# Derek-TH-Wang/OpenRoboRL

Hardware: AMD Instinct MI355X
Metric: env steps/sec at N parallel robots (higher is better)
Workload: dtype f32

## Files before the change

openroborl_amd/csrc/orr_device.h:

```cpp
#pragma once
#include <hip/hip_runtime.h>
#include <stddef.h>
#include <stdint.h>

#include "../../include/openroborl_hip.h"

#define ORR_PI_F 3.14159265358979323846f
#define WSYNC()                             \
  do {                                      \
    asm volatile("" ::: "memory");          \
    __builtin_amdgcn_wave_barrier();        \
    asm volatile("" ::: "memory");          \
  } while (0)

namespace orr {

constexpr int kLanes = 16;
constexpr int kRPW = 64 / kLanes;
constexpr int kMaxRows = 28;
constexpr int kHead = 308;

struct DevClip {
  const float* frames;
  const float* vels;
  int F, flags;
  double dt_d, dur_d;
  double sim_dt_d;
  float cdp[3];
  float cdh;
};
static_assert(sizeof(DevClip) == 64, "clip header = 16 words");

struct ModelHot {
  float jdir[12], joff[12];
  float joint_lo[12], joint_hi[12];
  float joint_pos[12][3];
  float toe_pos[4][3];
  float shank_pos[4][3];
  float lower_com[4][3];
  float init_quat[4];
  float toe_radius, shank_radius;
  float contact_cfm, contact_erp_dt;
};
static_assert(sizeof(ModelHot) == 512, "LDS budget: 4 robots per wave, two waves per SIMD = 20 KB per wave (DESIGN.md section 3)");
struct ModelCold {
  float init_pos[3];
  float foot_friction;
  float init_motor_angles[12], motor_dir[12], motor_offset[12];
  int joint_of_motor[12];
  float kp[12], kd[12];
  float tau_sign[12];
  float tau_sign_motor[12];
  float link_com[12][3];
  float default_joints[12];
  int num_fall;
  int fall_body[ORR_MAX_FALL_PROXIES];
  float fall_pos[ORR_MAX_FALL_PROXIES][3];
  float fall_radius[ORR_MAX_FALL_PROXIES];
  float mass[13];
  float inertia[13][6];
  float inertia_pa[13][6];
  int group[13];
  int friction_anchor;
};
struct alignas(16) DevModel {
  ModelHot hot;
  ModelCold cold;
};
static_assert(sizeof(DevModel) % 16 == 0 && offsetof(DevModel, hot) == 0, "16-byte pieces");
constexpr int kModelLdsWords = (int)(sizeof(ModelHot) / 4);

struct DevTables {
  DevModel model[ORR_MAX_ROBOT_TYPES];
  DevClip clip[ORR_MAX_CLIPS];
  int clip_set[ORR_MAX_ROBOT_TYPES][ORR_MAX_CLIPS];
  int clip_set_n[ORR_MAX_ROBOT_TYPES];
  int* clip_log;
  float clip_switch[ORR_MAX_ROBOT_TYPES][2];
  orr_task_noise noise;
};
static_assert(sizeof(orr_task_noise) == 32, "the noise variants read it as eight words");

struct ReplayArgs {
  const float* traj;
  const float* eff;
  const uint8_t* fall;
  float* tau_out;
  const float* uniforms;
};

struct KParams {
  orr_config cfg;
  float fb[3], fa[3];
  const DevTables* tab;
  float* state;
  long long* counters;
  float* ep_log;
  int ep_log_cap;
  int simds;
  int anchor_on;
#ifdef ORR_WAVE_TIMELINE
  long long* wave_times;
// ... 332 lines not shown
```

openroborl_amd/csrc/orr_env_kernels.h:

```cpp
#pragma once
#if defined(ORR_PHASE_TIMERS) && !defined(ORR_WAVE_TIMELINE)
#define ORR_WAVE_TIMELINE 1
#endif
#ifndef ORR_TU_MAIN
#undef ORR_PHASE_TIMERS
#endif
#include <hip/hip_runtime.h>
#include <type_traits>
#include <math.h>
#include <stdint.h>
#include <stdio.h>
#include <stdlib.h>
#include <string.h>

#include "orr_device.h"

#ifdef ORR_PHASE_TIMERS
__device__ long long g_phase_cycles[orr::kPhaseSlots];
__device__ long long g_wave_phases[2048 * 40];
#define PT_INIT() do { if (threadIdx.x == 0) { for (int i_ = 0; i_ < orr::kPhaseSlots; i_++) S.pt_acc[i_] = 0; S.pt_last = clock64(); } } while (0)
#define PT(k) do { if (threadIdx.x == 0) { const long long t_ = clock64(); S.pt_acc[k] += t_ - S.pt_last; S.pt_last = clock64(); } } while (0)
#define PT_FLUSH() do { if (threadIdx.x == 0 && blockIdx.x == gridDim.x / 2) for (int i_ = 0; i_ < orr::kPhaseSlots; i_++) atomicAdd((unsigned long long*)&g_phase_cycles[i_], (unsigned long long)S.pt_acc[i_]); \
                        if (threadIdx.x == 0 && blockIdx.x < 2048) for (int i_ = 0; i_ < orr::kPhaseSlots; i_++) g_wave_phases[blockIdx.x * 40 + i_] = S.pt_acc[i_]; } while (0)
#else
// ... 79 lines not shown
  }
  for (int i = lane; i < kMaxRows * kWStride; i += kLanes) (&S.ph.sub.W[0][0])[i] = 0.0f;
  WSYNC();
  LegConst K;
  load_leg_const(P, S, lane, K);
  {
    float rel[4], Rb[9];
    base_rotation(S, lane, rel, Rb);
  }
  AnchorState AS = {{0.0f, 0.0f, 0.0f}, {0.0f, 0.0f, 0.0f}, 0};
  bool anchor_robot = false;
  const int aleg = lane < 4 ? lane : (lane < 8 ? lane - 4 : (lane - 8) >> 1);
  if constexpr (ANCHOR) {
    static_assert(kLanes == 16, "ANCHOR: aleg indexes the record's four cached points by the 16-lane row layout");
    anchor_robot = model_cold(P, geti(S, O(ROBOT_TYPE)))->friction_anchor != 0;
    const float* an = rec + O(ANCHOR) + 6 * aleg;
    AS.la[0] = an[0]; AS.la[1] = an[1]; AS.la[2] = an[2]; AS.wb[0] = an[3]; AS.wb[1] = an[4]; AS.wb[2] = an[5];
    AS.valid = anchor_robot ? __float_as_int(rec[O(ANCHOR_VALID) + aleg]) : 0;
  }
  auto store_anchor = [&]() __attribute__((always_inline)) {
    if constexpr (ANCHOR) {
      if (valid && lane >= 4 && lane < 8) {
        float* an = rec + O(ANCHOR) + 6 * aleg;
        an[0] = AS.la[0]; an[1] = AS.la[1]; an[2] = AS.la[2]; an[3] = AS.wb[0]; an[4] = AS.wb[1]; an[5] = AS.wb[2];
        rec[O(ANCHOR_VALID) + aleg] = __int_as_float(AS.valid);
      }
    }
  };
  PT(0);

  if (MODE == 1) {
    if (lane < 12) {
      const ColdPtr mc = model_cold(P, geti(S, O(ROBOT_TYPE)));
      const int j = mc->joint_of_motor[lane];
      S.tau[j] = mc->tau_sign_motor[lane] * actions[(size_t)robot * 12 + lane];
    }
    WSYNC();
    int fall = 0;
    OwnCoord X;
    load_own_coord(S, lane, X);
    int limit_idle = 0;
    for (int s = 0; s < nsub; s++) {
      fall = physics_substep<ANCHOR>(P, S, K, lane, sub, true, X, limit_idle, ANCHOR ? &AS : nullptr, anchor_robot);
      float rel[4], Rb[9];
      base_rotation(S, lane, rel, Rb);
      WSYNC();
    }
    if (valid && lane == 0 && done_out) done_out[robot] = (uint8_t)fall;
    store_robot(rec, S, lane, valid);
    store_anchor();
    return;
  }

  const int ml = lane < 12 ? lane : 0;
  const ColdPtr mc = model_cold(P, geti(S, O(ROBOT_TYPE)));
  const int mj = mc->joint_of_motor[ml];
  const float m_off = mc->motor_offset[ml], m_dir = mc->motor_dir[ml], m_kp = mc->kp[ml], m_kd = mc->kd[ml];
  const float m_tsign = mc->tau_sign_motor[ml], m_init = mc->init_motor_angles[ml];
  ctrl_obs(P, rec, S, lane);
  float act_in = actions[(size_t)robot * 12 + ml];
  {
    const bool bad_act = !(fabsf(act_in) < 1e30f);
    if (bad_act) act_in = 0.0f;
    const bool any_bad = ((__ballot(bad_act) >> (sub * kLanes)) & ((1ull << (kLanes - 1)) * 2ull - 1ull)) != 0ull;
    if (lane == 0 && any_bad) S.s[kHead - 1] = 1.0f;
  }
  if (lane < 12) {
    const float act = act_in + m_init;
    S.s[O(LAST_ACTION) + lane] = act;
    float x1 = S.s[O(XHIST) + lane], x2 = S.s[O(XHIST) + 12 + lane], y1 = S.s[O(YHIST) + lane], y2 = S.s[O(YHIST) + 12 + lane];
    if (geti(S, O(STATE_ACTION_COUNTER)) == 0) {
      const float d = map_pi(S.co[lane]);
      x1 = x2 = y1 = y2 = d;
    }
    const float y = act * P.fb[0] + (x1 * P.fb[1] + x2 * P.fb[2]) - (y1 * P.fa[1] + y2 * P.fa[2]);
    S.s[O(XHIST) + 12 + lane] = x1; S.s[O(XHIST) + lane] = act;
    S.s[O(YHIST) + 12 + lane] = y1; S.s[O(YHIST) + lane] = y;
    S.s[O(ACTION) + lane] = y;
  }
  WSYNC();
  PT(1);
  int fall = 0;
  const float inv_repeat = 1.0f / (float)c.action_repeat;
  const RingLatency rlat = ring_latency(P, S);
  const float m_gain = m_tsign * S.s[O(STRENGTH) + ml];
  const float m_target = S.s[O(ACTION) + ml], m_prev = S.s[O(FILTER_ACTION) + ml];
  const bool m_has_prev = geti(S, O(FILTER_VALID)) != 0;
  int action_counter = geti(S, O(STATE_ACTION_COUNTER));
  RingCursor ring = {geti(S, O(RING_HEAD)), geti(S, O(RING_LEN))};
  OwnCoord X;
  load_own_coord(S, lane, X);
  int limit_idle = 0;
  const int prio_phase = WPE == 2 ? (int)(((unsigned)wave_id / (unsigned)(P.simds > 0 ? P.simds : 1)) & 1u) : 0;
  const bool prio_turns = WPE == 2 && ((((unsigned)gridDim.x + (unsigned)(P.simds > 0 ? P.simds : 1) - 1u) /
                                        (unsigned)(P.simds > 0 ? P.simds : 1)) & 1u) == 0u;
  float co_own = S.co[ml], qm_c = (S.s[O(Q) + mj] - m_off) * m_dir, qdm_c = S.s[O(QD) + mj] * m_dir;
  for (int sstep = 0; sstep < c.action_repeat; sstep++) {
    constexpr int kPrioTurn = 4, kPrioHi = 1, kPrioOffset = 1, kPrioEqualFrom = 1000;
    if (WPE == 2 && prio_turns) { if (sstep < kPrioEqualFrom && ((((sstep + kPrioOffset) / kPrioTurn) ^ prio_phase) & 1)) __builtin_amdgcn_s_setprio(kPrioHi); else __builtin_amdgcn_s_setprio(0); }
    {
      const float lerp = (float)(sstep + 1) * inv_repeat;
      const float cur = map_pi(co_own);
      const float prev = m_has_prev ? m_prev : cur;
      float cmd = prev + lerp * (m_target - prev);
      cmd = fminf(fmaxf(cmd, cur - c.max_angle_change), cur + c.max_angle_change);
      S.tau[lane < 12 ? mj : lane] = m_gain * (-1.0f * (m_kp * (qm_c - cmd)) - m_kd * qdm_c);
    }
    WSYNC();
    action_counter++;
    PT(2);
    {
      RingFetch F;
      ring_prefetch(rlat, rec, ring, lane, F);
      if constexpr (MODE == 2) {
        const size_t slot = (size_t)robot * c.action_repeat + sstep;
        if (lane < 12 && valid) RP.tau_out[slot * 12 + lane] = S.tau[mj] * m_tsign;
        WSYNC();
        for (int i = lane; i < 37; i += kLanes) S.s[O(POS) + i] = RP.traj[slot * 37 + i];
        WSYNC();
        fall = RP.fall[robot];
      } else
      fall = physics_substep<ANCHOR>(P, S, K, lane, sub, sstep == c.action_repeat - 1, X, limit_idle, ANCHOR ? &AS : nullptr, anchor_robot);
      qm_c = (S.s[O(Q) + mj] - m_off) * m_dir;
      qdm_c = S.s[O(QD) + mj] * m_dir;
      ring_push_and_ctrl_obs(rec, S, lane, valid, F, ring, qm_c, &co_own);
    }
    PT(10);
  }
  if (WPE == 2) __builtin_amdgcn_s_setprio(3);
  const ResetConst RC = load_reset_const(P, S, lane);
  if (lane == 0) {
    seti(S, O(RING_HEAD), ring.head); seti(S, O(RING_LEN), ring.len);
    seti(S, O(STATE_ACTION_COUNTER), action_counter);
    seti(S, O(FILTER_VALID), 1);
    seti(S, O(STEP_COUNTER), geti(S, O(STEP_COUNTER)) + 1);
  }
  if (lane < 12) S.s[O(FILTER_ACTION) + lane] = m_target;
  WSYNC();
  sensors_push(S, lane, false);
  PT(11);
  const DevClip& clip = S.clip;
  double t = motion_time(P, S);
  double t_phase = t;
  bool switched = false;
  if constexpr (CLIPS) {
    if (t >= (double)clip_change) {
      typedef const int __attribute__((address_space(1)))* gip;
      typedef const float __attribute__((address_space(1)))* gfp;
      const int type = geti(S, O(ROBOT_TYPE));
      const int set_n = ((gip)&P.tab->clip_set_n[0])[type];
      const float sw_min = ((gfp)&P.tab->clip_switch[type][0])[0], sw_max = ((gfp)&P.tab->clip_switch[type][0])[1];
      if (set_n > 1 && sw_max < INFINITY) {
        float u4[4];
        philox_block(c.seed, (uint32_t)geti(S, O(ROBOT_INDEX)), (uint32_t)geti(S, O(EPISODE_IDX)), 8u + (uint32_t)geti(S, O(EP_STEP)), u4);
        const uint32_t m = (uint32_t)(u4[0] * 16777216.0f);
        const int k = (int)((m * (uint32_t)set_n) >> 24);
        const int id = ((gip)&P.tab->clip_set[type][0])[k];
        clip_change = clip_change_time(t, sw_min, sw_max, u4[1]);
        WSYNC();
        if (lane == 0) seti(S, O(CLIP_ID), id);
        const unsigned int* cg = reinterpret_cast<const unsigned int*>(&P.tab->clip[id]);
        unsigned int* cl = reinterpret_cast<unsigned int*>(&S.clip);
        if (lane < (int)(sizeof(DevClip) / 4)) cl[lane] = cg[lane];
        WSYNC();
        if (lane == 0) {
          S.s[O(TIME_OFFSET)] = u4[2] * (float)clip.dur_d;
          if (valid) rec[O(CLIP_CHANGE_TIME)] = clip_change;
        }
        WSYNC();
        t = motion_time(P, S);
        switched = true;
      }
    }
  }
  const double step_dt = clip.sim_dt_d * c.action_repeat;
  double tl = t;
  {
    const int k = lane - 1;
    const int steps = (k & 2) ? ((k & 1) ? c.tar_frame_steps[3] : c.tar_frame_steps[2]) : ((k & 1) ? c.tar_frame_steps[1] : c.tar_frame_steps[0]);
    if (lane >= 1 && lane <= 4) tl = t + steps * step_dt;
  }
  PoseLoads PL;
  sample_poses_issue(P, S, lane, tl, PL);
  float rew = calc_reward(P, S, lane, MODE == 2 ? RP.eff + (size_t)robot * 48 : nullptr);
  sample_poses_finish(P, S, lane, tl, true, PL);
  {
    const float ph = clip_phase(clip, t_phase);
    if (lane == 0) {
      bool sync_pos = (c.flags & ORR_FLAG_CYCLE_SYNC) && ph < S.s[O(PREV_PHASE)];
      if constexpr (CLIPS) {
        if (switched) {
          q_about_z(task_heading(S, &S.s[O(QUAT)]) - task_heading(S, &S.ph.end.pose[0][3]), &S.s[O(ORIGIN_ROT)]);
          sync_pos = true;
        }
      }
      if (sync_pos) {
        float pr[3];
        qrot(&S.ph.end.pose[0][0], &S.s[O(ORIGIN_ROT)], pr);
        S.s[O(ORIGIN_POS)] = S.s[O(POS)] - pr[0];
        S.s[O(ORIGIN_POS) + 1] = S.s[O(POS) + 1] - pr[1];
        S.s[O(ORIGIN_POS) + 2] = 0.0f;
      }
      S.s[O(PREV_PHASE)] = ph;
      float v[3];
      qrot(&S.ph.end.vel[0], &S.s[O(ORIGIN_ROT)], v); S.ph.end.vel[0] = v[0]; S.ph.end.vel[1] = v[1]; S.ph.end.vel[2] = v[2];
      qrot(&S.ph.end.vel[3], &S.s[O(ORIGIN_ROT)], v); S.ph.end.vel[3] = v[0]; S.ph.end.vel[4] = v[1]; S.ph.end.vel[5] = v[2];
    }
    WSYNC();
    apply_origin(S, lane, 5);
    for (int i = lane; i < 19; i += kLanes) S.s[O(REF_POSE) + i] = S.ph.end.pose[0][i];
    for (int i = lane; i < 18; i += kLanes) S.s[O(REF_VEL) + i] = S.ph.end.vel[i];
    WSYNC();
  }
  PT(12);
  int reason = 0;
// ... 124 lines not shown
```

openroborl_amd/csrc/orr_physics.h:

```cpp
#pragma once


__device__ __forceinline__ void chol6(const float A[36], float L[21], float invdiag[6]) {
#pragma unroll
  for (int i = 0; i < 6; i++) {
#pragma unroll
    for (int j = 0; j <= i; j++) {
      float s = A[i * 6 + j];
#pragma unroll
      for (int k = 0; k < j; k++) s -= L[i * (i + 1) / 2 + k] * L[j * (j + 1) / 2 + k];
      if (i == j) {
        const float rs = rsq(s);
        L[i * (i + 1) / 2 + j] = s * rs;
        invdiag[i] = rs;
      } else {
        L[i * (i + 1) / 2 + j] = s * invdiag[j];
      }
    }
  }
}
__device__ __forceinline__ void chol6_solve(const float L[21], const float invdiag[6], const float b[6], float x[6]) {
  float y[6];
#pragma unroll
  for (int i = 0; i < 6; i++) {
    float s = b[i];
#pragma unroll
    for (int k = 0; k < i; k++) s -= L[i * (i + 1) / 2 + k] * y[k];
    y[i] = s * invdiag[i];
  }
#pragma unroll
  for (int i = 5; i >= 0; i--) {
    float s = y[i];
#pragma unroll
    for (int k = i + 1; k < 6; k++) s -= L[k * (k + 1) / 2 + i] * x[k];
    x[i] = s * invdiag[i];
  }
}

typedef float pk2 __attribute__((ext_vector_type(2)));
__device__ __forceinline__ pk2 pk_nfma(pk2 a, float s, pk2 c) { return __builtin_elementwise_fma(-a, pk2{s, s}, c); }
struct Chol6Pk {
  float l10, l32, l54;
  pk2 c0a, c0b;
  pk2 c1a, c1b;
  pk2 c2b, c3b;
  float idg[6];
};
__device__ __forceinline__ void chol6_pk(float d0, float d1, float d3, float d5, float a10, pk2 d2a, pk2 d4a,
                                         pk2 a0a, pk2 a0b, pk2 a1a, pk2 a1b, pk2 a2b, pk2 a3b, Chol6Pk& F) {
  const float r0 = rsq(d0);
  const float l10 = a10 * r0;
  const pk2 c0a = a0a * r0, c0b = a0b * r0;
  d1 = fmaf(-l10, l10, d1);
  a1a = pk_nfma(c0a, l10, a1a); a1b = pk_nfma(c0b, l10, a1b);
  d2a = pk_nfma(c0a, c0a.x, d2a);
  d3 = fmaf(-c0a.y, c0a.y, d3);
  a2b = pk_nfma(c0b, c0a.x, a2b); a3b = pk_nfma(c0b, c0a.y, a3b);
  d4a = pk_nfma(c0b, c0b.x, d4a);
  d5 = fmaf(-c0b.y, c0b.y, d5);
  const float r1 = rsq(d1);
  const pk2 c1a = a1a * r1, c1b = a1b * r1;
  d2a = pk_nfma(c1a, c1a.x, d2a);
  d3 = fmaf(-c1a.y, c1a.y, d3);
  a2b = pk_nfma(c1b, c1a.x, a2b); a3b = pk_nfma(c1b, c1a.y, a3b);
  d4a = pk_nfma(c1b, c1b.x, d4a);
  d5 = fmaf(-c1b.y, c1b.y, d5);
  const float r2 = rsq(d2a.x);
  const float l32 = d2a.y * r2;
  const pk2 c2b = a2b * r2;
  d3 = fmaf(-l32, l32, d3);
  a3b = pk_nfma(c2b, l32, a3b);
  d4a = pk_nfma(c2b, c2b.x, d4a);
  d5 = fmaf(-c2b.y, c2b.y, d5);
  const float r3 = rsq(d3);
  const pk2 c3b = a3b * r3;
  d4a = pk_nfma(c3b, c3b.x, d4a);
  d5 = fmaf(-c3b.y, c3b.y, d5);
  const float r4 = rsq(d4a.x);
  const float l54 = d4a.y * r4;
  d5 = fmaf(-l54, l54, d5);
  F.idg[0] = r0; F.idg[1] = r1; F.idg[2] = r2; F.idg[3] = r3; F.idg[4] = r4; F.idg[5] = rsq(d5);
  F.l10 = l10; F.l32 = l32; F.l54 = l54;
  F.c0a = c0a; F.c0b = c0b; F.c1a = c1a; F.c1b = c1b; F.c2b = c2b; F.c3b = c3b;
}
__device__ __forceinline__ void chol6_solve_pk(const Chol6Pk& F, float b0, float b1, pk2 b23, pk2 b45, float x[6]) {
  float y[6];
  y[0] = b0 * F.idg[0];
  b1 = fmaf(-F.l10, y[0], b1); b23 = pk_nfma(F.c0a, y[0], b23); b45 = pk_nfma(F.c0b, y[0], b45);
  y[1] = b1 * F.idg[1];
  b23 = pk_nfma(F.c1a, y[1], b23); b45 = pk_nfma(F.c1b, y[1], b45);
  y[2] = b23.x * F.idg[2];
  b23.y = fmaf(-F.l32, y[2], b23.y); b45 = pk_nfma(F.c2b, y[2], b45);
  y[3] = b23.y * F.idg[3];
  b45 = pk_nfma(F.c3b, y[3], b45);
  y[4] = b45.x * F.idg[4];
  b45.y = fmaf(-F.l54, y[4], b45.y);
  y[5] = b45.y * F.idg[5];
  x[5] = y[5] * F.idg[5];
  x[4] = fmaf(-F.l54, x[5], y[4]) * F.idg[4];
  x[3] = fmaf(-F.c3b.y, x[5], fmaf(-F.c3b.x, x[4], y[3])) * F.idg[3];
  x[2] = fmaf(-F.c2b.y, x[5], fmaf(-F.c2b.x, x[4], fmaf(-F.l32, x[3], y[2]))) * F.idg[2];
  x[1] = fmaf(-F.c1b.y, x[5], fmaf(-F.c1b.x, x[4], fmaf(-F.c1a.y, x[3], fmaf(-F.c1a.x, x[2], y[1])))) * F.idg[1];
  x[0] = fmaf(-F.c0b.y, x[5], fmaf(-F.c0b.x, x[4], fmaf(-F.c0a.y, x[3], fmaf(-F.c0a.x, x[2], fmaf(-F.l10, x[1], y[0]))))) * F.idg[0];
}

#ifdef ORR_TU_STEP_W2
constexpr bool kCarrySubtreeMass = false, kOwnLegFactor = false, kPackedVelocityUpdate = false;
#define ORR_COMMON(x) (x)
#define ORR_RARE(x) (x)
#else
constexpr bool kCarrySubtreeMass = true, kOwnLegFactor = true, kPackedVelocityUpdate = true;
#define ORR_COMMON(x) __builtin_expect(!!(x), 1)
#define ORR_RARE(x) __builtin_expect(!!(x), 0)
#endif
struct LegConst {
  float r[3][3], jdir[3], joff[3];
  float com[3], m, Ic[6];
  float msub;
  float damp_l, damp_a;
  float jdir_own, joff_own;
  float int_c0, int_c1;
};
struct OwnCoord { float x0, x1; };
__device__ __forceinline__ void load_own_coord(const Shared& S, int lane, OwnCoord& X) {
  X.x0 = lane < 3 ? 0.0f : (lane < 6 ? S.s[O(POS) + lane - 3] : S.s[O(Q) + lane - 6]);
  X.x1 = lane < 2 ? S.s[O(Q) + 10 + lane] : 0.0f;
}
__device__ __forceinline__ float part_suffix_sum(float x);
__device__ static void load_leg_const(const KParams& P, const Shared& S, int lane, LegConst& K) {
  const int leg = lane & 3, part = (lane >> 2) & 3, own = 3 * leg + (part < 3 ? part : 2);
  const ColdPtr mc = model_cold(P, geti(S, O(ROBOT_TYPE)));
#pragma unroll
  for (int k = 0; k < 3; k++) {
    const int j = 3 * leg + k;
    const bool on = k <= part && part < 3;
#pragma unroll
    for (int i = 0; i < 3; i++) K.r[k][i] = on ? S.m.joint_pos[j][i] : 0.0f;
    K.jdir[k] = on ? S.m.jdir[j] : 0.0f;
    K.joff[k] = S.m.joff[j];
  }
  const bool real = part < 3, base = lane == 12;
  const int body = real ? own + 1 : 0;
#pragma unroll
  for (int i = 0; i < 3; i++) K.com[i] = real ? mc->link_com[own][i] : 0.0f;
  {
    const int g = mc->group[body];
    const float mr = S.s[O(MASS_RATIO) + g], ir = S.s[O(INERTIA_RATIO) + g];
    const float mass = mc->mass[body] * mr;
#pragma unroll
    for (int i = 0; i < 6; i++) K.Ic[i] = (real || base) ? mc->inertia[body][i] * ir + mc->inertia_pa[body][i] * mr : 0.0f;
    K.m = (real || base) ? mass : 0.0f;
    if (kCarrySubtreeMass) K.msub = part_suffix_sum(K.m);
  }
  K.jdir_own = real ? S.m.jdir[own] : 0.0f;
  K.joff_own = S.m.joff[own];
  K.damp_l = base ? S.s[O(BASE_DAMPING)] : 0.0f;
  K.damp_a = base ? S.s[O(BASE_DAMPING) + 1] : 0.0f;
  K.int_c0 = lane < 3 ? 0.0f : (lane < 6 ? 1.0f : S.m.jdir[lane < 6 ? 0 : lane - 6]);
  K.int_c1 = lane < 2 ? S.m.jdir[10 + lane] : 0.0f;
}


__device__ __forceinline__ void rot_sym_full(const float R[9], const float S[6], float O[6]) {
  float T[9];
#pragma unroll
  for (int i = 0; i < 3; i++) {
    T[3 * i] = R[3 * i] * S[0] + R[3 * i + 1] * S[3] + R[3 * i + 2] * S[4];
    T[3 * i + 1] = R[3 * i] * S[3] + R[3 * i + 1] * S[1] + R[3 * i + 2] * S[5];
    T[3 * i + 2] = R[3 * i] * S[4] + R[3 * i + 1] * S[5] + R[3 * i + 2] * S[2];
  }
  O[0] = T[0] * R[0] + T[1] * R[1] + T[2] * R[2];
  O[1] = T[3] * R[3] + T[4] * R[4] + T[5] * R[5];
  O[2] = T[6] * R[6] + T[7] * R[7] + T[8] * R[8];
  O[3] = T[0] * R[3] + T[1] * R[4] + T[2] * R[5];
  O[4] = T[0] * R[6] + T[1] * R[7] + T[2] * R[8];
  O[5] = T[3] * R[6] + T[4] * R[7] + T[5] * R[8];
}
__device__ __forceinline__ void spatial_inertia_mul(const float I[6], const float h[3], float m, const float w[3], const float v[3],
                                                    float oa[3], float ol[3]) {
  oa[0] = fmaf(I[0], w[0], fmaf(I[3], w[1], fmaf(I[4], w[2], fmaf(h[1], v[2], -h[2] * v[1]))));
  oa[1] = fmaf(I[3], w[0], fmaf(I[1], w[1], fmaf(I[5], w[2], fmaf(h[2], v[0], -h[0] * v[2]))));
  oa[2] = fmaf(I[4], w[0], fmaf(I[5], w[1], fmaf(I[2], w[2], fmaf(h[0], v[1], -h[1] * v[0]))));
  ol[0] = fmaf(m, v[0], fmaf(h[2], w[1], -h[1] * w[2]));
  ol[1] = fmaf(m, v[1], fmaf(h[0], w[2], -h[2] * w[0]));
  ol[2] = fmaf(m, v[2], fmaf(h[1], w[0], -h[0] * w[1]));
}

template <int AX, bool SAME_AXIS = false>
__device__ __forceinline__ void joint_down(const Shared& S, const LegConst& K, int k, int j, float sn, float cs, float Rw[9], float d[3],
                                           float Vw[3], float Vv[3], float Aa[3], float Al[3], float s[3], float sv[3], float& ad_out,
                                           float* c0 = nullptr) {
  const float ad = K.jdir[k] * S.s[O(QD) + j];
  ad_out = ad;
#pragma unroll
  for (int i = 0; i < 3; i++)
    d[i] = fmaf(Rw[3 * i], K.r[k][0], fmaf(Rw[3 * i + 1], K.r[k][1], fmaf(Rw[3 * i + 2], K.r[k][2], d[i])));
// ... 644 lines not shown
      else sb = bcast_lane<src>(__builtin_amdgcn_fmed3f(yA, loE, hiE), sub);
      yA = fmaf(AcA[r], sb, yp);
      lam[r] = sb;
      if (HAS_B) yB = fmaf(AcB[r], sb - old, yB);
      if (r >= 16 && r < 20) {
        constexpr int g = r >= 16 && r < 20 ? r - 16 : 0;
        const float d = sb - old;
        hiE = fmaf(mun[g], d, hiE); loE = fmaf(-mun[g], d, loE);
      }
    };
    static_for<0, 4>(rowA);
    if (HAS_B) {
      for_active_limit_rows(mask, [&](auto rc) __attribute__((always_inline)) {
        constexpr int r = decltype(rc)::value;
        const float old = lam[r];
        const float yp = fmaf(-AcB[r], old, yB);
        const float sb = dpp_bcast_max0<r>(yB, zero);
        yB = fmaf(AcB[r], sb, yp);
        lam[r] = sb;
        yA = fmaf(AcA[r], sb - old, yA);
      });
    }
    static_for<16, 28>(rowA);
  }
}

template <int K>
__device__ __forceinline__ float zero_in_lane(float x, int lane) {
  float o;
  asm("v_cmp_eq_u32 vcc, %2, %1\n\tv_cndmask_b32_e64 %0, %3, 0, vcc" : "=v"(o) : "v"(lane), "n"(K), "v"(x) : "vcc");
  return o;
}
template <bool HAS_B>
__device__ __forceinline__ void delassus_columns(const Shared& S, unsigned int mask, int lane, int sub, Row& A, Row& B, const ContactGeom& G,
                                                 float (&AcA)[kMaxRows], float (&AcB)[kMaxRows], float (&lam)[kMaxRows]) {
#pragma unroll
  for (int r = 0; r < kMaxRows; r++) {
    AcA[r] = 0.0f; AcB[r] = 0.0f;
    if (HAS_B || r < 4 || r >= 16) lam[r] = 0.0f;
  }
  auto finish = [&](auto rc, float a, float b) __attribute__((always_inline)) {
    constexpr int r = decltype(rc)::value;
    constexpr bool inB = r >= 4 && r < 16;
    constexpr int src = inB ? r : (r < 4 ? r : r - 12);
    const float l0 = bcast_lane<src>(inB ? B.lam : A.lam, sub);
    lam[r] = l0;
    A.w += a * l0;
    AcA[r] = inB ? -a * A.jdi : zero_in_lane<src>(-a * A.jdi, lane);
    if (r >= 16 && r < 20 && A.nrm_slot == r) A.lam_n = l0;
    if (HAS_B) {
      B.w += b * l0;
      AcB[r] = inB ? zero_in_lane<src>(-b * B.jdi, lane) : -b * B.jdi;
    }
    asm("" : "+v"(AcA[r]), "+v"(AcB[r]));
  };
  static_for<0, 4>([&](auto rc) __attribute__((always_inline)) {
    constexpr int r = decltype(rc)::value;
    finish(rc, A.wq[3 * r + 2], HAS_B ? B.wq[3 * r + 2] : 0.0f);
  });
  if (HAS_B) {
    for_active_limit_rows(mask, [&](auto rc) __attribute__((always_inline)) {
      constexpr int r = decltype(rc)::value;
      const float sg = bcast_lane<r>(B.jl[(r - 4) % 3], sub);
      finish(rc, sg * A.wq[r - 4], sg * B.wq[r - 4]);
    });
  }
  const unsigned int cm = (mask >> 16) & 0xFu;
  static_for<0, 4>([&](auto gc) __attribute__((always_inline)) {
    constexpr int g = decltype(gc)::value;
    if (ORR_COMMON((cm >> g) & 1u)) {
      float ax, ay, az, bx = 0.0f, by = 0.0f, bz = 0.0f;
      dpp_contact_triplet<4 + g>(G.rr0, G.rr1, G.rr2, G.c00, G.c01, G.c02, G.c10, G.c11, G.c12, G.c20, G.c21, G.c22, A.wa[0], A.wa[1], A.wa[2],
                                 A.wa[3], A.wa[4], A.wa[5], A.wq[3 * g], A.wq[3 * g + 1], A.wq[3 * g + 2], ax, ay, az);
      if (HAS_B)
        dpp_contact_triplet<4 + g>(G.rr0, G.rr1, G.rr2, G.c00, G.c01, G.c02, G.c10, G.c11, G.c12, G.c20, G.c21, G.c22, B.wa[0], B.wa[1], B.wa[2],
                                   B.wa[3], B.wa[4], B.wa[5], B.wq[3 * g], B.wq[3 * g + 1], B.wq[3 * g + 2], bx, by, bz);
      finish(std::integral_constant<int, 16 + g>{}, az, bz);
      finish(std::integral_constant<int, 20 + 2 * g>{}, ax, bx);
      finish(std::integral_constant<int, 21 + 2 * g>{}, ay, by);
    }
  });
}

template <bool ANCHOR = false>
__device__ static int physics_substep(const KParams& P, Shared& S, const LegConst& K, int lane, int sub, bool want_fall, OwnCoord& X,
                                      int& limit_idle, AnchorState* AS = nullptr, bool anchor_robot = false) {
  const orr_config& cfg = P.cfg;
  const float dt = cfg.sim_dt, inv_dt = 1.0f / cfg.sim_dt, erp_dt = cfg.contact_erp / cfg.sim_dt;
  int fp_body = 0, fp_n = 0;
  float fp_x = 0.0f, fp_y = 0.0f, fp_z = 0.0f, fp_r = 0.0f;
  if (ORR_RARE(want_fall)) {
    const ColdPtr mc = model_cold(P, geti(S, O(ROBOT_TYPE)));
    static_assert(ORR_MAX_FALL_PROXIES <= kLanes, "one fall proxy per lane");
    fp_body = mc->fall_body[lane]; fp_x = mc->fall_pos[lane][0]; fp_y = mc->fall_pos[lane][1]; fp_z = mc->fall_pos[lane][2]; fp_r = mc->fall_radius[lane];
    fp_n = mc->num_fall;
  }
  BaseFactor BF;
  leg_dynamics(P, S, K, lane, BF);
  WSYNC();
  PT(3);
  asm volatile("" : "+v"(fp_n));
  int fall = 0;
  if (ORR_RARE(want_fall)) {
    bool hit = false;
    if (lane < fp_n) {
      const int b = fp_body;
      const float* Rw = b == 0 ? S.Rb : S.ph.sub.dyn.lc[b - 1].Rw;
      const float oz = b == 0 ? S.s[O(POS) + 2] : S.ph.sub.dyn.lc[b - 1].ow[2];
      const float wz = Rw[6] * fp_x + Rw[7] * fp_y + Rw[8] * fp_z;
      hit = (oz + wz - fp_r) < cfg.contact_margin;
    }
    fall = ((__ballot(hit) >> (sub * kLanes)) & ((1ull << (kLanes - 1)) * 2ull - 1ull)) != 0ull;
  }
  PT(4);

  Row A, B;
  const bool rowlane = lane < 16;
  ContactGeom G;
  row_setup_bank_a<ANCHOR>(S, cfg, rowlane ? (lane < 4 ? lane : lane + 12) : 0, rowlane, dt, inv_dt, erp_dt, A, G, AS, anchor_robot);
  unsigned long long balB = 0ull;
  if (ORR_COMMON(limit_idle > 0)) {
    limit_idle--;
    B.active = false;
  } else {
    float margin = 1e30f;
    row_setup_limit(S, cfg, (rowlane && lane >= 4) ? lane : 4, rowlane && lane >= 4, inv_dt, erp_dt, B, &margin);
    balB = __ballot(B.active);
    const float steps_f = (rowlane && lane >= 4) ? margin * __builtin_amdgcn_rcpf(cfg.max_coord_velocity * dt) - 1.0f : 1e30f;
    int idle = 0;
    if (__ballot(steps_f < 1.0f) == 0ull) idle = 1;
    if (__ballot(steps_f < 2.0f) == 0ull) idle = 2;
    if (__ballot(steps_f < 4.0f) == 0ull) idle = 4;
    if (__ballot(steps_f < 8.0f) == 0ull) idle = 8;
    if (__ballot(steps_f < 16.0f) == 0ull) idle = 16;
    limit_idle = idle;
  }
  const unsigned long long balA = __ballot(A.active);
  const bool anyB = balB != 0ull;
  unsigned int mask = 0;
#pragma unroll
  for (int g = 0; g < kRPW; g++) {
    const unsigned int a = (unsigned int)(balA >> (g * kLanes)) & 0xFFFFu, b2 = (unsigned int)(balB >> (g * kLanes)) & 0xFFF0u;
    mask |= (a & 0xFu) | ((a >> 4) << 16) | b2;
  }
  PT(5);
  row_response(S, cfg, A, rowlane ? (lane < 4 ? lane : lane + 12) : 0, BF);
  if (ORR_RARE(anyB)) row_response(S, cfg, B, (rowlane && lane >= 4) ? lane : kMaxRows, BF);
  WSYNC();
  PT(6);
  float AcA[kMaxRows], AcB[kMaxRows], lam[kMaxRows];
  if (ORR_RARE(anyB)) {
    delassus_columns<true>(S, mask, lane, sub, A, B, G, AcA, AcB, lam);
    PT(7);
    pgs_sweeps<true>(cfg.solver_iters, mask, lane, sub, A, B, AcA, AcB, lam);
    PT(34);
  } else {
    delassus_columns<false>(S, mask, lane, sub, A, B, G, AcA, AcB, lam);
    PT(7);
    pgs_sweeps<false>(cfg.solver_iters, mask, lane, sub, A, B, AcA, AcB, lam);
  }
  PT(8);
  {
#pragma unroll
    for (int g = 0; g < 4; g++) {
      S.s[O(LAMBDA) + 3 * g] = lam[16 + g];
      S.s[O(LAMBDA) + 3 * g + 1] = lam[20 + 2 * g];
      S.s[O(LAMBDA) + 3 * g + 2] = lam[21 + 2 * g];
    }
  }
  float v0, v1;
  {
    const int k1 = lane + 16 < 18 ? lane + 16 : 0;
    const int k0 = lane < 18 ? lane : 0;
    float du0 = 0.0f, du1 = 0.0f;
    if constexpr (kPackedVelocityUpdate) {
      static_assert(kLanes + 16 + (kMaxRows - 1) * kWStride < (kMaxRows + 1) * kWStride, "the second word of the last row's pair lies inside W");
      v2f du = {0.0f, 0.0f};
      const float* const wk = &S.ph.sub.W[0][k0];
      auto row_pair = [&](auto rc) __attribute__((always_inline)) {
        constexpr int r = decltype(rc)::value;
        return v2f{wk[r * kWStride], wk[r * kWStride + 16]};
      };
      v2f wr[kMaxRows];
      static_for<0, 4>([&](auto rc) __attribute__((always_inline)) { wr[decltype(rc)::value] = row_pair(rc); });
      static_for<16, 28>([&](auto rc) __attribute__((always_inline)) { wr[decltype(rc)::value] = row_pair(rc); });
      asm volatile("" : "+v"(wr[0]), "+v"(wr[1]), "+v"(wr[2]), "+v"(wr[3]), "+v"(wr[16]), "+v"(wr[17]), "+v"(wr[18]), "+v"(wr[19]),
                        "+v"(wr[20]), "+v"(wr[21]), "+v"(wr[22]), "+v"(wr[23]), "+v"(wr[24]), "+v"(wr[25]), "+v"(wr[26]), "+v"(wr[27]));
      auto add_row = [&](auto rc) __attribute__((always_inline)) { du += wr[decltype(rc)::value] * lam[decltype(rc)::value]; };
      static_for<0, 4>(add_row);
      if (ORR_RARE(anyB)) {
        for_active_limit_rows(mask, [&](auto rc) __attribute__((always_inline)) { du += row_pair(rc) * lam[decltype(rc)::value]; });
      }
      static_for<16, 28>(add_row);
      du0 = du.x; du1 = du.y;
    } else {
      auto add_row = [&](auto rc) __attribute__((always_inline)) {
        constexpr int r = decltype(rc)::value;
        du0 += S.ph.sub.W[r][k0] * lam[r];
        du1 += S.ph.sub.W[r][k1] * lam[r];
      };
      static_for<0, 4>(add_row);
      if (anyB) {
        for_active_limit_rows(mask, add_row);
      }
      static_for<16, 28>(add_row);
    }
    const float vmax = cfg.max_coord_velocity;
    v0 = __builtin_amdgcn_fmed3f(S.ustar[k0] + du0, -vmax, vmax);
    v1 = __builtin_amdgcn_fmed3f(S.ustar[k1] + du1, -vmax, vmax);
  }
  {
    const float w0 = bcast_lane<0>(v0, sub), w1 = bcast_lane<1>(v0, sub), w2 = bcast_lane<2>(v0, sub);
    const float ww = w0 * w0 + w1 * w1 + w2 * w2, h2 = 0.25f * dt * dt * ww;
    const float sc = 0.5f * dt * fmaf(h2, fmaf(h2, fmaf(h2, -1.0f / 5040.0f, 1.0f / 120.0f), -1.0f / 6.0f), 1.0f);
    const float ch = fmaf(h2, fmaf(h2, fmaf(h2, fmaf(h2, 1.0f / 40320.0f, -1.0f / 720.0f), 1.0f / 24.0f), -0.5f), 1.0f);
    const float dq[4] = {w0 * sc, w1 * sc, w2 * sc, ch};
    float qn[4];
    qmul(dq, &S.s[O(QUAT)], qn);
    const float nn = rsq(qn[0] * qn[0] + qn[1] * qn[1] + qn[2] * qn[2] + qn[3] * qn[3]);
    X.x0 = fmaf(dt * v0, K.int_c0, X.x0);
    X.x1 = fmaf(dt * v1, K.int_c1, X.x1);
    float* const dump = &S.ustar[22];
    float* const pv0 = &S.s[lane < 3 ? O(ANGVEL) + lane : (lane < 6 ? O(LINVEL) + lane - 3 : O(QD) + lane - 6)];
    float* const px0 = lane < 3 ? dump : &S.s[lane < 6 ? O(POS) + lane - 3 : O(Q) + lane - 6];
    float* const pv1 = lane < 2 ? &S.s[O(QD) + 10 + lane] : dump;
    float* const px1 = lane < 2 ? &S.s[O(Q) + 10 + lane] : dump;
    float* const pq = lane < 4 ? &S.s[O(QUAT) + lane] : dump;
    WSYNC();
    *pv0 = lane < 6 ? v0 : v0 * K.int_c0;
    *px0 = X.x0;
    *pv1 = v1 * K.int_c1;
    *px1 = X.x1;
    *pq = pick4(lane, qn[0], qn[1], qn[2], qn[3]) * nn;
  }
  WSYNC();
  PT(9);
  return fall;
}
```

openroborl_amd/csrc/orr_robot_io.h:

```cpp
#pragma once

typedef float f4 __attribute__((ext_vector_type(4)));
__device__ static void load_robot(const KParams& P, const float* rec, Shared& S, int lane) {
  {
    static_assert(kHead % 4 == 0 && ORR_STATE_STRIDE % 4 == 0, "16-byte pieces");
    typedef const f4 __attribute__((address_space(1))) * g4ptr;
    const g4ptr src = (g4ptr)reinterpret_cast<const f4*>(rec);
    f4* dst = reinterpret_cast<f4*>(S.s);
    constexpr int kQ = kHead / 4, kIt = (kQ + kLanes - 1) / kLanes;
    f4 tmp[kIt];
#pragma unroll
    for (int k = 0; k < kIt; k++) { const int q = lane + k * kLanes; tmp[k] = src[q < kQ ? q : kQ - 1]; }
#pragma unroll
    for (int k = 0; k < kIt; k++) { const int q = lane + k * kLanes; if (q < kQ) dst[q] = tmp[k]; }
  }
  WSYNC();
  const DevModel& gm = P.tab->model[geti(S, O(ROBOT_TYPE))];
  {
    static_assert(sizeof(DevClip) % 4 == 0 && sizeof(DevClip) / 4 <= kLanes, "one word of the clip header per lane");
    const unsigned int* cg = reinterpret_cast<const unsigned int*>(&P.tab->clip[geti(S, O(CLIP_ID))]);
    unsigned int* cl = reinterpret_cast<unsigned int*>(&S.clip);
    if (lane < (int)(sizeof(DevClip) / 4)) cl[lane] = cg[lane];
  }
  {
    typedef const f4 __attribute__((address_space(1))) * g4ptr;
    static_assert(sizeof(ModelHot) % (16 * kLanes) == 0 && alignof(DevModel) >= 16, "whole 16-byte rows of the hot model per lane");
    const g4ptr mp = (g4ptr)reinterpret_cast<const f4*>(&gm.hot);
    f4* dst = reinterpret_cast<f4*>(&S.m);
    constexpr int kIter = (int)(sizeof(ModelHot) / 16) / kLanes;
    f4 tmp[kIter];
#pragma unroll
    for (int k = 0; k < kIter; k++) tmp[k] = mp[lane + k * kLanes];
#pragma unroll
    for (int k = 0; k < kIter; k++) dst[lane + k * kLanes] = tmp[k];
  }
  WSYNC();
}

__device__ static void store_robot(float* rec, const Shared& S, int lane, bool valid) {
  if (valid) {
    typedef f4 __attribute__((address_space(1))) * g4ptr;
    const g4ptr dst = (g4ptr)reinterpret_cast<f4*>(rec);
    const f4* src = reinterpret_cast<const f4*>(S.s);
    constexpr int kQ = O(RING) / 4;
#pragma unroll
    for (int k = 0; k < (kQ + kLanes - 1) / kLanes; k++) { const int q = lane + k * kLanes; if (q < kQ) dst[q] = src[q]; }
    if (lane < O(RING) - 4 * kQ) rec[4 * kQ + lane] = S.s[4 * kQ + lane];
  }
}

__device__ static void ctrl_obs(const KParams& P, const float* rec, Shared& S, int lane) {
  const float lat = S.s[O(LATENCY)], dt = P.cfg.sim_dt;
  const int len = geti(S, O(RING_LEN)), head = geti(S, O(RING_HEAD));
  int k0 = 0, k1 = 0;
  float al = 0.0f;
  if (!(lat <= 0.0f || len == 1)) {
    int n = (int)(lat / dt);
    if (n + 1 >= len) { k0 = k1 = len - 1; }
    else { k0 = n; k1 = n + 1; al = (lat - n * dt) / dt; }
  }
  const int i0 = (head - k0 + 2 * ORR_RING_DEPTH) % ORR_RING_DEPTH, i1 = (head - k1 + 2 * ORR_RING_DEPTH) % ORR_RING_DEPTH;
  for (int i = lane; i < 19; i += kLanes) {
    float e0 = rec[O(RING) + i0 * ORR_RING_ENTRY + i], e1 = rec[O(RING) + i1 * ORR_RING_ENTRY + i];
    S.co[i] = (k0 == k1) ? e0 : (1.0f - al) * e0 + al * e1;
  }
  WSYNC();
}

__device__ __forceinline__ void base_rotation(Shared& S, int lane, float rel[4], float Rb[9]) {
  float qi[4];
  qinv(S.m.init_quat, qi);
  qmul(&S.s[O(QUAT)], qi, rel);
  q_to_mat(rel, Rb);
#pragma unroll
  for (int i = 0; i < 9; i++) S.Rb[i] = Rb[i];
}

struct ResetConst {
  int j;
  float off, dir;
  float init;
  float p0;
};
__device__ __forceinline__ ResetConst load_reset_const(const KParams& P, const Shared& S, int lane) {
  const ColdPtr mc = model_cold(P, geti(S, O(ROBOT_TYPE)));
  const int ml = lane < 12 ? lane : 0;
  return ResetConst{mc->joint_of_motor[ml], mc->motor_offset[ml], mc->motor_dir[ml], mc->init_motor_angles[ml], mc->init_pos[lane < 3 ? lane : 0]};
}

__device__ static void receive_obs(const KParams& P, float* rec, Shared& S, int lane, bool valid, const ResetConst& RC, float* entry = nullptr) {
  const int head = (geti(S, O(RING_HEAD)) + 1) % ORR_RING_DEPTH, len = geti(S, O(RING_LEN));
  float rel[4], Rb[9], rate[3];
  base_rotation(S, lane, rel, Rb);
  mtv3(Rb, &S.s[O(ANGVEL)], rate);
  for (int i = lane; i < ORR_RING_ENTRY; i += kLanes) {
    float val = 0.0f;
    if (i < 12) {
      static_assert(kLanes >= 12, "the first pass of the loop covers the twelve motors");
      val = (S.s[O(Q) + RC.j] - RC.off) * RC.dir;
    } else if (i < 16) {
      val = i == 12 ? rel[0] : (i == 13 ? rel[1] : (i == 14 ? rel[2] : rel[3]));
    } else if (i < 19) {
      val = i == 16 ? rate[0] : (i == 17 ? rate[1] : rate[2]);
    }
    if (valid) rec[O(RING) + head * ORR_RING_ENTRY + i] = val;
    if (entry) entry[i] = val;
  }
  WSYNC();
  if (lane == 0) {
    seti(S, O(RING_HEAD), head);
    seti(S, O(RING_LEN), len + 1 > ORR_RING_DEPTH ? ORR_RING_DEPTH : len + 1);
  }
  WSYNC();
}

struct RingFetch {
  float e0[2], e1[2];
  float al;
  bool new0, new1, same;
};
struct RingLatency {
  int n;
  float al;
  bool none;
};
__device__ __forceinline__ RingLatency ring_latency(const KParams& P, const Shared& S) {
  const float lat = S.s[O(LATENCY)], dt = P.cfg.sim_dt;
  RingLatency L;
  L.none = lat <= 0.0f;
  L.n = (int)(lat / dt);
  L.al = (lat - L.n * dt) / dt;
  return L;
}
struct RingCursor { int head, len; };
__device__ __forceinline__ int ring_wrap_up(int i) { return i >= ORR_RING_DEPTH ? i - ORR_RING_DEPTH : i; }
__device__ __forceinline__ int ring_wrap_down(int i) { return i < 0 ? i + ORR_RING_DEPTH : i; }
__device__ __forceinline__ void ring_prefetch(const RingLatency& L, const float* rec, const RingCursor& C, int lane, RingFetch& F) {
  const int head = ring_wrap_up(C.head + 1);
  const int len = C.len + 1 > ORR_RING_DEPTH ? ORR_RING_DEPTH : C.len + 1;
  int k0 = 0, k1 = 0;
  F.al = 0.0f;
  if (!(L.none || len == 1)) {
    if (L.n + 1 >= len) { k0 = k1 = len - 1; }
    else { k0 = L.n; k1 = L.n + 1; F.al = L.al; }
  }
  F.same = k0 == k1; F.new0 = k0 == 0; F.new1 = k1 == 0;
  const int i0 = ring_wrap_down(head - k0), i1 = ring_wrap_down(head - k1);
  const float* p0 = rec + O(RING) + i0 * ORR_RING_ENTRY;
  const float* p1 = rec + O(RING) + i1 * ORR_RING_ENTRY;
  const int hi = lane < 3 ? 16 + lane : lane;
  F.e0[0] = p0[lane]; F.e0[1] = p0[hi];
  F.e1[0] = p1[lane]; F.e1[1] = p1[hi];
}
__device__ __forceinline__ void ring_push_and_ctrl_obs(float* rec, Shared& S, int lane, bool valid, const RingFetch& F, RingCursor& C,
                                                       float mang, float* co_own = nullptr) {
  static_assert(ORR_RING_ENTRY == 20, "lane mapping below assumes 20-word entries");
  C.head = ring_wrap_up(C.head + 1);
  C.len = C.len + 1 > ORR_RING_DEPTH ? ORR_RING_DEPTH : C.len + 1;
  float rel[4], Rb[9], rate[3];
  base_rotation(S, lane, rel, Rb);
  mtv3(Rb, &S.s[O(ANGVEL)], rate);
  const float va = lane < 12 ? mang : pick4(lane, rel[0], rel[1], rel[2], rel[3]);
  const float vb = pick4(lane, rate[0], rate[1], rate[2], 0.0f);
  const float a0 = F.new0 ? va : F.e0[0], a1 = F.new1 ? va : F.e1[0];
  const float b0 = F.new0 ? vb : F.e0[1], b1 = F.new1 ? vb : F.e1[1];
  const float co_a = F.same ? a0 : (1.0f - F.al) * a0 + F.al * a1;
  S.co[lane] = co_a;
  if (co_own) *co_own = co_a;
  S.co[lane < 3 ? 16 + lane : 19] = F.same ? b0 : (1.0f - F.al) * b0 + F.al * b1;
  WSYNC();
  float* dst = rec + O(RING) + C.head * ORR_RING_ENTRY;
  if (valid) {
    dst[lane] = va;
    dst[lane < 4 ? 16 + lane : lane] = lane < 4 ? vb : va;
  }
}
```

Before: 21.73 million.

## Trim per-substep ring observation work and reuse integrated base state

The ring cursor and latency offsets are kept in words instead of entries, which removes a multiply and simplifies wrap and clamp logic in the substep loop. The second half of each ring entry (rates) is now fetched and interpolated into the shared control observation only on the last substep, because only the motor-angle part is consumed by intermediate substeps via co_own. Physics now hands back the freshly integrated quaternion and angular velocity in registers so the observation code does not reread them from LDS. Uninitialised fall-proxy locals and branch hints shave further instructions. The risk is that S.co lanes are left stale on intermediate substeps if anything else reads them there.

```diff
diff --git a/openroborl_amd/csrc/orr_device.h b/openroborl_amd/csrc/orr_device.h
--- a/openroborl_amd/csrc/orr_device.h
+++ b/openroborl_amd/csrc/orr_device.h
@@ -18,6 +18,13 @@
 constexpr int kLanes = 16;
 constexpr int kRPW = 64 / kLanes;
 constexpr int kMaxRows = 28;
+#ifdef ORR_TU_STEP_W2
+#define ORR_COMMON(x) (x)
+#define ORR_RARE(x) (x)
+#else
+#define ORR_COMMON(x) __builtin_expect(!!(x), 1)
+#define ORR_RARE(x) __builtin_expect(!!(x), 0)
+#endif
 constexpr int kHead = 308;
 
 struct DevClip {
diff --git a/openroborl_amd/csrc/orr_env_kernels.h b/openroborl_amd/csrc/orr_env_kernels.h
--- a/openroborl_amd/csrc/orr_env_kernels.h
+++ b/openroborl_amd/csrc/orr_env_kernels.h
@@ -185,12 +185,13 @@
   PT(1);
   int fall = 0;
   const float inv_repeat = 1.0f / (float)c.action_repeat;
-  const RingLatency rlat = ring_latency(P, S);
   const float m_gain = m_tsign * S.s[O(STRENGTH) + ml];
   const float m_target = S.s[O(ACTION) + ml], m_prev = S.s[O(FILTER_ACTION) + ml];
   const bool m_has_prev = geti(S, O(FILTER_VALID)) != 0;
   int action_counter = geti(S, O(STATE_ACTION_COUNTER));
-  RingCursor ring = {geti(S, O(RING_HEAD)), geti(S, O(RING_LEN))};
+  RingLatency rlat = ring_latency(P, S);
+  ring_latency_words(rlat);
+  RingCursor ring = ring_words(geti(S, O(RING_HEAD)), geti(S, O(RING_LEN)));
   OwnCoord X;
   load_own_coord(S, lane, X);
   int limit_idle = 0;
@@ -214,7 +215,9 @@
     PT(2);
     {
       RingFetch F;
-      ring_prefetch(rlat, rec, ring, lane, F);
+      const bool last = sstep == c.action_repeat - 1;
+      ring_prefetch(rlat, rec, ring, lane, last, F);
+      IntegratedBase IB;
       if constexpr (MODE == 2) {
         const size_t slot = (size_t)robot * c.action_repeat + sstep;
         if (lane < 12 && valid) RP.tau_out[slot * 12 + lane] = S.tau[mj] * m_tsign;
@@ -222,18 +225,20 @@
         for (int i = lane; i < 37; i += kLanes) S.s[O(POS) + i] = RP.traj[slot * 37 + i];
         WSYNC();
         fall = RP.fall[robot];
-      } else
-      fall = physics_substep<ANCHOR>(P, S, K, lane, sub, sstep == c.action_repeat - 1, X, limit_idle, ANCHOR ? &AS : nullptr, anchor_robot);
+      } else {
+        fall = physics_substep<ANCHOR>(P, S, K, lane, sub, last, X, limit_idle, ANCHOR ? &AS : nullptr, anchor_robot, &IB);
+      }
       qm_c = (S.s[O(Q) + mj] - m_off) * m_dir;
       qdm_c = S.s[O(QD) + mj] * m_dir;
-      ring_push_and_ctrl_obs(rec, S, lane, valid, F, ring, qm_c, &co_own);
+      ring_push_and_ctrl_obs(rec, S, lane, valid, last, F, ring, qm_c, MODE == 2 ? nullptr : IB.q, MODE == 2 ? nullptr : IB.w, &co_own);
     }
     PT(10);
   }
   if (WPE == 2) __builtin_amdgcn_s_setprio(3);
   const ResetConst RC = load_reset_const(P, S, lane);
   if (lane == 0) {
-    seti(S, O(RING_HEAD), ring.head); seti(S, O(RING_LEN), ring.len);
+    const RingCursor rc = ring_entries(ring);
+    seti(S, O(RING_HEAD), rc.head); seti(S, O(RING_LEN), rc.len);
     seti(S, O(STATE_ACTION_COUNTER), action_counter);
     seti(S, O(FILTER_VALID), 1);
     seti(S, O(STEP_COUNTER), geti(S, O(STEP_COUNTER)) + 1);
diff --git a/openroborl_amd/csrc/orr_physics.h b/openroborl_amd/csrc/orr_physics.h
--- a/openroborl_amd/csrc/orr_physics.h
+++ b/openroborl_amd/csrc/orr_physics.h
@@ -106,12 +106,8 @@
 
 #ifdef ORR_TU_STEP_W2
 constexpr bool kCarrySubtreeMass = false, kOwnLegFactor = false, kPackedVelocityUpdate = false;
-#define ORR_COMMON(x) (x)
-#define ORR_RARE(x) (x)
 #else
 constexpr bool kCarrySubtreeMass = true, kOwnLegFactor = true, kPackedVelocityUpdate = true;
-#define ORR_COMMON(x) __builtin_expect(!!(x), 1)
-#define ORR_RARE(x) __builtin_expect(!!(x), 0)
 #endif
 struct LegConst {
   float r[3][3], jdir[3], joff[3];
@@ -922,13 +918,14 @@
   });
 }
 
+struct IntegratedBase { float q[4], w[3]; };
 template <bool ANCHOR = false>
 __device__ static int physics_substep(const KParams& P, Shared& S, const LegConst& K, int lane, int sub, bool want_fall, OwnCoord& X,
-                                      int& limit_idle, AnchorState* AS = nullptr, bool anchor_robot = false) {
+                                      int& limit_idle, AnchorState* AS = nullptr, bool anchor_robot = false, IntegratedBase* out = nullptr) {
   const orr_config& cfg = P.cfg;
   const float dt = cfg.sim_dt, inv_dt = 1.0f / cfg.sim_dt, erp_dt = cfg.contact_erp / cfg.sim_dt;
-  int fp_body = 0, fp_n = 0;
-  float fp_x = 0.0f, fp_y = 0.0f, fp_z = 0.0f, fp_r = 0.0f;
+  int fp_body, fp_n = __builtin_nondeterministic_value(fp_n);
+  float fp_x, fp_y, fp_z, fp_r;
   if (ORR_RARE(want_fall)) {
     const ColdPtr mc = model_cold(P, geti(S, O(ROBOT_TYPE)));
     static_assert(ORR_MAX_FALL_PROXIES <= kLanes, "one fall proxy per lane");
@@ -1071,7 +1068,14 @@
     *px0 = X.x0;
     *pv1 = v1 * K.int_c1;
     *px1 = X.x1;
-    *pq = pick4(lane, qn[0], qn[1], qn[2], qn[3]) * nn;
+    if (out) {
+      const float q0 = qn[0] * nn, q1 = qn[1] * nn, q2 = qn[2] * nn, q3 = qn[3] * nn;
+      *pq = pick4(lane, q0, q1, q2, q3);
+      out->q[0] = q0; out->q[1] = q1; out->q[2] = q2; out->q[3] = q3;
+      out->w[0] = w0; out->w[1] = w1; out->w[2] = w2;
+    } else {
+      *pq = pick4(lane, qn[0], qn[1], qn[2], qn[3]) * nn;
+    }
   }
   WSYNC();
   PT(9);
diff --git a/openroborl_amd/csrc/orr_robot_io.h b/openroborl_amd/csrc/orr_robot_io.h
--- a/openroborl_amd/csrc/orr_robot_io.h
+++ b/openroborl_amd/csrc/orr_robot_io.h
@@ -67,14 +67,15 @@
   WSYNC();
 }
 
-__device__ __forceinline__ void base_rotation(Shared& S, int lane, float rel[4], float Rb[9]) {
+__device__ __forceinline__ void base_rotation_of(Shared& S, const float q[4], float rel[4], float Rb[9]) {
   float qi[4];
   qinv(S.m.init_quat, qi);
-  qmul(&S.s[O(QUAT)], qi, rel);
+  qmul(q, qi, rel);
   q_to_mat(rel, Rb);
 #pragma unroll
   for (int i = 0; i < 9; i++) S.Rb[i] = Rb[i];
 }
+__device__ __forceinline__ void base_rotation(Shared& S, int lane, float rel[4], float Rb[9]) { base_rotation_of(S, &S.s[O(QUAT)], rel, Rb); }
 
 struct ResetConst {
   int j;
@@ -132,44 +133,56 @@
   L.al = (lat - L.n * dt) / dt;
   return L;
 }
+constexpr int kRingWords = ORR_RING_DEPTH * ORR_RING_ENTRY;
 struct RingCursor { int head, len; };
-__device__ __forceinline__ int ring_wrap_up(int i) { return i >= ORR_RING_DEPTH ? i - ORR_RING_DEPTH : i; }
-__device__ __forceinline__ int ring_wrap_down(int i) { return i < 0 ? i + ORR_RING_DEPTH : i; }
-__device__ __forceinline__ void ring_prefetch(const RingLatency& L, const float* rec, const RingCursor& C, int lane, RingFetch& F) {
-  const int head = ring_wrap_up(C.head + 1);
-  const int len = C.len + 1 > ORR_RING_DEPTH ? ORR_RING_DEPTH : C.len + 1;
-  int k0 = 0, k1 = 0;
-  F.al = 0.0f;
-  if (!(L.none || len == 1)) {
-    if (L.n + 1 >= len) { k0 = k1 = len - 1; }
-    else { k0 = L.n; k1 = L.n + 1; F.al = L.al; }
+__device__ __forceinline__ RingCursor ring_words(int head, int len) { return RingCursor{head * ORR_RING_ENTRY, len * ORR_RING_ENTRY}; }
+__device__ __forceinline__ RingCursor ring_entries(const RingCursor& C) {
+  return RingCursor{(int)((unsigned)C.head / (unsigned)ORR_RING_ENTRY), (int)((unsigned)C.len / (unsigned)ORR_RING_ENTRY)};
+}
+__device__ __forceinline__ void ring_latency_words(RingLatency& L) {
+  const int n = L.none || L.n < 0 ? 0 : L.n;
+  L.n = (n < ORR_RING_DEPTH ? n : ORR_RING_DEPTH) * ORR_RING_ENTRY;
+}
+__device__ __forceinline__ int ring_wrap_up(int i) { return i >= kRingWords ? i - kRingWords : i; }
+__device__ __forceinline__ int ring_wrap_down(int i) { return i < 0 ? i + kRingWords : i; }
+__device__ __forceinline__ void ring_prefetch(const RingLatency& L, const float* rec, const RingCursor& C, int lane, bool last, RingFetch& F) {
+  const int head = ring_wrap_up(C.head + ORR_RING_ENTRY);
+  const int len = C.len + ORR_RING_ENTRY > kRingWords ? kRingWords : C.len + ORR_RING_ENTRY;
+  const int oldest = len - ORR_RING_ENTRY;
+  const int k0 = L.n < oldest ? L.n : oldest;
+  const int k1 = L.none ? 0 : (L.n + ORR_RING_ENTRY < oldest ? L.n + ORR_RING_ENTRY : oldest);
+  F.al = (!L.none && L.n + ORR_RING_ENTRY < len) ? L.al : 0.0f;
+  F.same = k0 == k1; F.new0 = k0 == 0; F.new1 = k1 == 0;
+  const unsigned int i0 = (unsigned int)ring_wrap_down(head - k0), i1 = (unsigned int)ring_wrap_down(head - k1);
+  const float* const ring = rec + O(RING);
+  F.e0[0] = ring[i0 + (unsigned int)lane];
+  F.e1[0] = ring[i1 + (unsigned int)lane];
+  if (ORR_RARE(last)) {
+    const unsigned int hi = lane < 3 ? 16u + (unsigned int)lane : (unsigned int)lane;
+    F.e0[1] = ring[i0 + hi];
+    F.e1[1] = ring[i1 + hi];
   }
-  F.same = k0 == k1; F.new0 = k0 == 0; F.new1 = k1 == 0;
-  const int i0 = ring_wrap_down(head - k0), i1 = ring_wrap_down(head - k1);
-  const float* p0 = rec + O(RING) + i0 * ORR_RING_ENTRY;
-  const float* p1 = rec + O(RING) + i1 * ORR_RING_ENTRY;
-  const int hi = lane < 3 ? 16 + lane : lane;
-  F.e0[0] = p0[lane]; F.e0[1] = p0[hi];
-  F.e1[0] = p1[lane]; F.e1[1] = p1[hi];
 }
-__device__ __forceinline__ void ring_push_and_ctrl_obs(float* rec, Shared& S, int lane, bool valid, const RingFetch& F, RingCursor& C,
-                                                       float mang, float* co_own = nullptr) {
+__device__ __forceinline__ void ring_push_and_ctrl_obs(float* rec, Shared& S, int lane, bool valid, bool last, const RingFetch& F, RingCursor& C,
+                                                       float mang, const float* q, const float* w, float* co_own = nullptr) {
   static_assert(ORR_RING_ENTRY == 20, "lane mapping below assumes 20-word entries");
-  C.head = ring_wrap_up(C.head + 1);
-  C.len = C.len + 1 > ORR_RING_DEPTH ? ORR_RING_DEPTH : C.len + 1;
+  C.head = ring_wrap_up(C.head + ORR_RING_ENTRY);
+  C.len = C.len + ORR_RING_ENTRY > kRingWords ? kRingWords : C.len + ORR_RING_ENTRY;
   float rel[4], Rb[9], rate[3];
-  base_rotation(S, lane, rel, Rb);
-  mtv3(Rb, &S.s[O(ANGVEL)], rate);
+  base_rotation_of(S, q ? q : &S.s[O(QUAT)], rel, Rb);
+  mtv3(Rb, w ? w : &S.s[O(ANGVEL)], rate);
   const float va = lane < 12 ? mang : pick4(lane, rel[0], rel[1], rel[2], rel[3]);
   const float vb = pick4(lane, rate[0], rate[1], rate[2], 0.0f);
   const float a0 = F.new0 ? va : F.e0[0], a1 = F.new1 ? va : F.e1[0];
-  const float b0 = F.new0 ? vb : F.e0[1], b1 = F.new1 ? vb : F.e1[1];
   const float co_a = F.same ? a0 : (1.0f - F.al) * a0 + F.al * a1;
-  S.co[lane] = co_a;
   if (co_own) *co_own = co_a;
-  S.co[lane < 3 ? 16 + lane : 19] = F.same ? b0 : (1.0f - F.al) * b0 + F.al * b1;
+  if (ORR_RARE(last)) {
+    const float b0 = F.new0 ? vb : F.e0[1], b1 = F.new1 ? vb : F.e1[1];
+    S.co[lane] = co_a;
+    S.co[lane < 3 ? 16 + lane : 19] = F.same ? b0 : (1.0f - F.al) * b0 + F.al * b1;
+  }
   WSYNC();
-  float* dst = rec + O(RING) + C.head * ORR_RING_ENTRY;
+  float* const dst = rec + O(RING) + (unsigned int)C.head;
   if (valid) {
     dst[lane] = va;
     dst[lane < 4 ? 16 + lane : lane] = lane < 4 ? vb : va;
```

Result: no change. 21.91 million (median of 6 runs) (+0.8%).
